# NVIDIA/DeepLearningExamples

Measured on AMD Instinct MI355X. Metric: training samples/sec, higher is better.
Workload: dtype bf16; 1 GPU; ResNet-50 v1.5 (PyTorch/Classification/ConvNets) synthetic ImageNet 224x224, label smoothing 0.1, SGD momentum 0.875 (BASELINE.json configs[1]); batch_per_gpu=256, global_batch=256, layout=NHWC, hip_graph=False, parallelism=single GPU

## Files before the change

deeplearningexamples_amd/_cabi.py:

```python
import ctypes
import os

import torch

_HERE = os.path.dirname(os.path.abspath(__file__))
LIB_PATH = os.environ.get("DLE_LIB_PATH") or os.path.join(_HERE, "lib", "libdle_mi355x.so")

F32, F16, BF16 = 0, 1, 2
ACT_NONE, ACT_RELU, ACT_GELU, ACT_RELU_BWD, ACT_ADD, ACT_GELU_BWD, ACT_TANH, ACT_TANH_BWD = 0, 1, 2, 3, 4, 5, 6, 7
ACT_ADD_MASKED, ACT_MUL, ACT_GELU_DAUX = 8, 9, 10

_DT = {torch.float32: F32, torch.float16: F16, torch.bfloat16: BF16}

c_void_p, c_int, c_i64, c_float = ctypes.c_void_p, ctypes.c_int, ctypes.c_int64, ctypes.c_float
c_u64 = ctypes.c_uint64

_SIGS = {
    "dle_last_error": (ctypes.c_char_p, []),
    "dle_abi_version": (c_int, []),
    "dle_device_check": (c_int, [c_int, ctypes.c_char_p, c_int]),
    "dle_dot_interact_out_width": (c_int, [c_int, c_int]),
    "dle_dot_interact_fwd": (c_int, [c_void_p, c_void_p, c_int, c_int, c_int, c_int, c_int, c_void_p]),
    "dle_dot_interact_bwd": (c_int, [c_void_p, c_void_p, c_void_p, c_void_p, c_int, c_int, c_int, c_int,
                                     c_int, c_void_p]),
    "dle_dot_interact_bwd_checked": (c_int, [c_void_p, c_void_p, c_void_p, c_void_p, c_int, c_int, c_int, c_int,
                                             c_int, c_void_p, c_void_p]),
    "dle_dlrm_gather_interact_try": (c_int, [c_void_p] * 6 + [c_i64, c_int, c_int, c_int, c_void_p]),
    "dle_emb_gather_fwd": (c_int, [c_void_p, c_void_p, c_void_p, c_void_p, c_void_p, c_i64, c_int, c_int,
                                   c_int, c_i64, c_void_p]),
    "dle_emb_offset_indices": (c_int, [c_void_p, c_void_p, c_void_p, c_void_p, c_i64, c_int, c_void_p]),
    "dle_emb_grad_values": (c_int, [c_void_p, c_void_p, c_void_p, c_i64, c_int, c_void_p]),
    "dle_emb_sparse_sgd": (c_int, [c_void_p, c_void_p, c_void_p, c_void_p, c_float, c_void_p, c_void_p,
                                   c_i64, c_int, c_int, c_i64, c_int, c_void_p]),
    "dle_emb_small_table_mask": (c_int, [c_void_p, c_int, c_int, c_void_p]),
    "dle_emb_sgd_dedup": (c_int, [c_void_p, c_void_p, c_void_p, c_void_p, c_void_p, c_void_p, c_void_p,
                                  c_void_p, c_float, c_void_p, c_void_p, c_i64, c_int, c_int, c_i64, c_int,
                                  c_void_p]),
    "dle_emb_sgd_dedup_ws": (c_int, [c_void_p, c_void_p, c_void_p, c_void_p, c_void_p, c_void_p, c_void_p,
                                     c_void_p, c_float, c_void_p, c_void_p, c_i64, c_int, c_int, c_i64, c_int,
                                     c_void_p, c_i64, c_void_p]),
    "dle_emb_onehot_workspace_bytes": (c_i64, [c_int, c_i64]),
    "dle_emb_sgd_workspace_bytes": (c_i64, [c_void_p, c_int, c_int, c_i64]),
    "dle_emb_onehot_try": (c_int, [c_void_p, c_void_p, c_void_p, c_void_p, c_float, c_void_p, c_void_p, c_void_p, c_void_p,
                                   c_void_p, c_int, c_i64, c_int, c_int, c_i64, c_int, c_void_p, c_i64, c_void_p]),
    "dle_emb_onehot_partials": (c_int, [c_void_p, c_void_p, c_void_p, c_void_p, c_void_p, c_void_p, c_int, c_i64, c_int, c_int,
                                        c_i64, c_int, c_void_p, c_i64, c_void_p, c_void_p]),
    "dle_emb_adam_workspace_bytes": (c_i64, [c_void_p, c_int, c_int, c_i64]),
    "dle_emb_adam_dedup_ws": (c_int, [c_void_p] * 9 + [c_float, c_void_p, c_void_p, c_void_p, c_float, c_float, c_float, c_i64,
                                      c_int, c_int, c_i64, c_int, c_void_p, c_i64, c_void_p]),
    "dle_cast_rows": (c_int, [c_void_p, c_void_p, c_i64, c_int, c_int, c_i64, c_i64, c_int, c_int, c_void_p]),
    "dle_bce_logits": (c_int, [c_void_p, c_void_p, c_void_p, c_void_p, c_void_p, c_i64, c_i64, c_int, c_void_p]),
    "dle_conv1x1_bnbwd_dgrad": (c_int, [c_void_p] * 16 + [c_i64, c_int, c_int, c_int, c_int, c_void_p]),
    "dle_conv1x1_bnbwd_groups": (c_int, [c_int]),
    "dle_conv1x1_bnbwd_dgrad_wgrad": (c_int, [c_void_p] * 15 + [c_i64, c_void_p, c_void_p, c_void_p, c_i64, c_int, c_int, c_int, c_int,
                                              c_void_p]),
    "dle_conv1x1_bnbwd_wgrad_workspace": (c_i64, [c_int, c_int]),
    "dle_gemm_expand_masked_bnred": (c_int, [c_void_p] * 10 + [c_i64, c_int, c_int, c_int, c_i64, c_i64, c_i64, c_int, c_int, c_void_p]),
    "dle_bn_bwd_finish": (c_int, [c_void_p, c_int, c_int, c_void_p, c_void_p, c_int, c_void_p]),
    "dle_gemm_colsum": (c_int, [c_void_p, c_void_p, c_void_p, c_void_p, c_void_p, c_int, c_int, c_int, c_i64, c_i64, c_i64, c_int,
                                c_int, c_int, c_void_p, c_i64, c_void_p]),
    "dle_head_bce_workspace_bytes": (c_i64, [c_i64, c_int]),
    "dle_head_bce_fwd_bwd": (c_int, [c_void_p, c_void_p, c_void_p, c_void_p, c_void_p, c_void_p, c_void_p, c_void_p, c_void_p,
                                     c_void_p, c_void_p, c_void_p, c_i64, c_i64, c_int, c_i64, c_i64, c_int, c_void_p]),
    "dle_amp_update_scale": (c_int, [c_void_p, c_void_p, c_void_p, c_void_p, c_float, c_float, c_int, c_int,
                                     c_void_p]),
    "dle_check_nonfinite": (c_int, [c_void_p, c_void_p, c_i64, c_int, c_void_p]),
    "dle_axpby_f32": (c_int, [c_void_p, c_void_p, c_void_p, c_float, c_float, c_i64, c_void_p]),
    "dle_act_bwd": (c_int, [c_void_p, c_void_p, c_void_p, c_i64, c_int, c_int, c_void_p]),
    "dle_relu_bwd": (c_int, [c_void_p, c_void_p, c_void_p, c_i64, c_int, c_i64, c_i64, c_i64, c_int, c_void_p]),
    "dle_gemm": (c_int, [c_void_p, c_void_p, c_void_p, c_void_p, c_void_p, c_void_p, c_int, c_int, c_int,
                         c_i64, c_i64, c_i64, c_int, c_int, c_int, c_int, c_int, c_int, c_int, c_float,
                         c_void_p, c_i64, c_void_p]),
    "dle_conv2d_fwd": (c_int, [c_void_p, c_void_p, c_void_p, c_void_p] + [c_int] * 12 + [c_void_p]),
    "dle_conv2d_fwd_affine": (c_int, [c_void_p] * 6 + [c_int] * 11 + [c_void_p]),
    "dle_conv3x3_affine_launch_count": (c_i64, []),
    "dle_conv2d_grouped_fwd_affine": (c_int, [c_void_p] * 5 + [c_int] * 9 + [c_void_p]),
    "dle_se_gate": (c_int, [c_void_p] * 6 + [c_int] * 5 + [c_void_p]),
    "dle_se_apply": (c_int, [c_void_p] * 4 + [c_i64, c_int, c_int, c_int, c_int, c_void_p]),
    "dle_conv2d_dgrad": (c_int, [c_void_p, c_void_p, c_void_p, c_void_p] + [c_int] * 10 + [c_void_p]),
    "dle_conv2d_wgrad": (c_int, [c_void_p, c_void_p, c_void_p] + [c_int] * 12 + [c_void_p, c_i64, c_void_p]),
    "dle_nchw_to_nhwc": (c_int, [c_void_p, c_void_p, c_i64, c_int, c_i64, c_int, c_int, c_void_p]),
    "dle_gemm_expand_add_up2": (c_int, [c_void_p, c_void_p, c_void_p, c_void_p, c_int, c_int, c_int, c_i64, c_i64, c_i64, c_i64, c_int,
                                        c_int, c_int, c_int, c_void_p]),
    "dle_conv1x1_bnload_groups": (c_int, [c_int, c_int, c_int]),
    "dle_conv1x1_bnload_fwd": (c_int, [c_void_p] * 11 + [c_i64, c_int, c_int, c_int, c_int, c_void_p]),
    "dle_bn_relu_maxpool_fwd": (c_int, [c_void_p] * 8 + [c_int, c_int, c_int, c_int, c_int, c_void_p]),
    "dle_wgrad1x1_workspace": (c_i64, []),
    "dle_wgrad1x1_mode": (c_int, [c_int]),
    "dle_wgrad1x1_workspace_for": (c_i64, [c_int, c_int, c_int]),
    "dle_gemm8_mode": (c_int, [c_int]),
    "dle_gemm8_min_items": (c_int, [c_int]),
    "dle_gemm8_launch_count": (c_i64, []),
    "dle_wgrad1x1_try": (c_int, [c_void_p, c_void_p, c_void_p, c_int, c_int, c_int, c_int, c_int, c_void_p, c_i64, c_void_p]),
    "dle_conv3x3_wgrad_workspace": (c_i64, []),
    "dle_conv3x3_wgrad_mode": (c_int, [c_int]),
    "dle_stem_conv7_groups": (c_int, [c_int, c_int]),
    "dle_stem_conv7_fwd": (c_int, [c_void_p, c_void_p, c_void_p, c_void_p, c_i64, c_int, c_int, c_int, c_int, c_void_p]),
    "dle_stem_conv7_wgrad_workspace": (c_i64, [c_int, c_int]),
    "dle_stem_conv7_wgrad": (c_int, [c_void_p, c_void_p, c_void_p, c_void_p, c_i64, c_int, c_int, c_int, c_int, c_int, c_void_p]),
    "dle_stem_pack_weight": (c_int, [c_void_p, c_void_p, c_int, c_void_p]),
    "dle_bn_workspace_bytes": (c_i64, [c_i64, c_int]),
    "dle_bn_fwd_stats": (c_int, [c_void_p, c_i64, c_int, c_float, c_float, c_void_p, c_void_p, c_void_p, c_void_p,
                                 c_void_p, c_i64, c_int, c_void_p]),
    "dle_conv2d_fwd_colstats": (c_int, [c_void_p, c_void_p, c_void_p] + [c_int] * 10 + [c_void_p, c_i64, c_void_p, c_void_p]),
    "dle_bn_stats_from_partials": (c_int, [c_void_p, c_int, c_i64, c_int, c_float, c_float, c_void_p, c_void_p, c_void_p,
                                           c_void_p, c_void_p, c_i64, c_void_p]),
    "dle_bn_fwd_apply": (c_int, [c_void_p] * 8 + [c_i64, c_int, c_int, c_int, c_void_p]),
    "dle_rccl_available": (c_int, []),
    "dle_rccl_unique_id": (c_int, [c_void_p]),
# ... 278 lines not shown
```

deeplearningexamples_amd/convnets/resnet.py:

```python
from contextlib import nullcontext as _nullcontext
from typing import List

import os

import torch
from torch import nn

from .. import _cabi as C
from .. import functional as F

LAYERS, WIDTHS, EXPANSION = [3, 4, 6, 3], [64, 128, 256, 512], 4


def _conv(cin, cout, k, stride, device):
    m = nn.Conv2d(cin, cout, kernel_size=k, stride=stride, padding=(k - 1) // 2, bias=False, device=device)
    nn.init.kaiming_normal_(m.weight, mode="fan_in", nonlinearity="relu")
    m.weight.data = m.weight.data.contiguous(memory_format=torch.channels_last)
    return m


def _bn(c, device, zero_init=False):
    m = nn.BatchNorm2d(c, device=device)
    nn.init.constant_(m.weight, 0 if zero_init else 1)
    nn.init.constant_(m.bias, 0)
    return m


class Deferred:
    __slots__ = ("unit", "t", "mean", "rstd", "residual", "y")

    def __init__(self, unit, t, mean, rstd, residual):
        self.unit, self.t, self.mean, self.rstd, self.residual, self.y = unit, t, mean, rstd, residual, None

    def residual_args(self):
        r = self.residual
        if isinstance(r, Deferred):
            return r.t, (r.mean, r.rstd, r.unit.bn.weight.data, r.unit.bn.bias.data)
        return r, None

    def _done(self, y, mask):
        u = self.unit
        u.saved = (u.saved[0], self.t, mask, self.mean, self.rstd)
        self.y = y

    def materialize(self):
        if self.y is None:
            u = self.unit
            res, res_bn = self.residual_args()
            y, mask = F.bn_fwd_apply(self.t, self.mean, self.rstd, u.bn.weight.data, u.bn.bias.data, residual=res,
                                     relu=u.relu, want_mask=True, residual_bn=res_bn)
            self._done(y, mask)
        return self.y


class ConvBN:

    def __init__(self, conv: nn.Conv2d, bn: nn.BatchNorm2d, name_conv: str, name_bn: str, relu: bool):
        self.conv, self.bn, self.name_conv, self.name_bn, self.relu = conv, bn, name_conv, name_bn, relu
        self.k = conv.kernel_size[0]
        self.stride, self.pad = conv.stride[0], conv.padding[0]
        self.cin, self.cout = conv.in_channels, conv.out_channels
        self.w16 = None
        self.gw = self.ggamma = self.gbeta = None
        self.saved = None
        self.w2 = self.gw_flat = None
        self.wgrad_stream = None
        self.fuse_bnbwd = os.environ.get("DLE_RN50_FUSE_BNBWD", "1") != "0"
        self.fuse_bnbwd_wgrad = os.environ.get("DLE_RN50_FUSE_BNBWD_WGRAD", "1") != "0"
        self.reduce_done = False
        self.keepalive = None

    def forward(self, x, residual=None, defer=False):
        t = None
        if isinstance(x, Deferred):
            d, r = x, None
            if self.k == 1 and self.stride == 1 and d.unit.relu and d.y is None:
                res, res_bn = d.residual_args()
                r = F.conv1x1_bnload_fwd(d.t, res, self.w16, d.mean, d.rstd, d.unit.bn.weight.data, d.unit.bn.bias.data,
                                         self.bn.running_mean, self.bn.running_var, eps=self.bn.eps, momentum=self.bn.momentum,
                                         res_bn=res_bn)
            if r is not None:
                t, x, bits, mean, rstd = r
                d._done(x, bits)
            else:
                x = d.materialize()
        if t is None:
            if x.shape[-1] == 4:
                t, mean, rstd = F.stem_conv_fwd_bnstats(x, self.w2, self.bn.running_mean, self.bn.running_var, eps=self.bn.eps,
                                                        momentum=self.bn.momentum)
            else:
                t, mean, rstd = F.conv2d_fwd_bnstats(x, self.w16, self.stride, self.pad, self.bn.running_mean,
                                                     self.bn.running_var, eps=self.bn.eps, momentum=self.bn.momentum)
        if defer:
            self.saved = (x, t, None, mean, rstd)
            return Deferred(self, t, mean, rstd, residual)
        if isinstance(residual, Deferred):
            d = Deferred(self, t, mean, rstd, residual)
            self.saved = (x, t, None, mean, rstd)
            return d.materialize()
        y, mask = F.bn_fwd_apply(t, mean, rstd, self.bn.weight.data, self.bn.bias.data, residual=residual,
                                 relu=self.relu, want_mask=True)
        self.saved = (x, t, mask, mean, rstd)
        return y

    def forward_eval(self, x, residual=None):
        t = F.stem_conv_fwd(x, self.w2, want_stats=False)[0] if x.shape[-1] == 4 else F.conv2d_fwd(x, self.w16, self.stride, self.pad)
        rstd = torch.rsqrt(self.bn.running_var + self.bn.eps)
        y, _ = F.bn_fwd_apply(t, self.bn.running_mean, rstd, self.bn.weight.data, self.bn.bias.data, residual=residual,
                              relu=self.relu, want_mask=False)
        return y

    def backward(self, dy, need_dx=True, dx_addend=None, dy_mask=None, compact_dx=False, bnred=None, pooled=None):
        x, t, mask, mean, rstd = self.saved
        self.saved = None
        self.saved_c = x.shape[-1]
        rmask = mask if self.relu else dy_mask
        n, h, w, c = x.shape
        reduce_done, self.reduce_done = self.reduce_done, False
        fused = None
        wgrad_done = False
        if self.fuse_bnbwd and self.k == 1 and self.stride == 1 and need_dx and dx_addend is None:
            b2 = None
            if bnred is not None and bnred.saved is not None and bnred.relu:
                b2 = (bnred.saved[1], bnred.saved[2], bnred.saved[3], bnred.saved[4], bnred.ggamma, bnred.gbeta)
            if self.fuse_bnbwd_wgrad and pooled is None and self.gw is not None:
                r = F.bn_bwd_conv1x1_dgrad_wgrad(dy, t, mean, rstd, self.bn.weight.data, self.ggamma, self.gbeta,
                                                 self.w16.view(self.cout, c), x, self.gw, relu_mask=rmask,
                                                 reduce_done=reduce_done, bnred=b2)
                if r is not None:
                    fused, wgrad_done = (None, r[0], r[1]), True
            if fused is None:
                fused = F.bn_bwd_conv1x1_dgrad(dy, t, mean, rstd, self.bn.weight.data, self.ggamma, self.gbeta,
                                               self.w16.view(self.cout, c), relu_mask=rmask, reduce_done=reduce_done, bnred=b2)
        gt = None
        if pooled is not None:
            if self.relu and not reduce_done:
                gt = F.pool_bn_bwd(pooled[0], pooled[1], t, mean, rstd, self.bn.weight.data, self.ggamma, self.gbeta, rmask)
            if gt is None:
                dy = F.maxpool_bwd(pooled[0], pooled[1], t.shape[1:3])
        if gt is not None:
            pass
        elif fused is not None:
            gt = fused[0]
            if fused[2]:
                bnred.reduce_done = True
        else:
            gt, _ = F.bn_bwd(dy, None, t, mean, rstd, self.bn.weight.data, self.ggamma, self.gbeta, relu_mask=rmask,
                             reduce_done=reduce_done)
        up2 = isinstance(dx_addend, tuple) and dx_addend[0] == "up2"
        masked = isinstance(dx_addend, tuple) and not up2
        ws = self.wgrad_stream if not wgrad_done else None
        if ws is not None:
            ws.wait_stream(torch.cuda.current_stream())
            self.keepalive.append((gt, x))
        with (torch.cuda.stream(ws) if ws is not None else _nullcontext()):
            if wgrad_done:
                pass
            elif c == 4:
                F.stem_conv_wgrad(gt, x, self.gw_flat)
            elif self.k == 1 and self.stride == 1:
                m = n * h * w
                if not F.wgrad1x1(gt.view(m, self.cout), x.view(m, c), self.gw.view(self.cout, c)):
                    F.gemm(gt.view(m, self.cout), x.view(m, c), self.cout, c, m, False, False, out=self.gw.view(self.cout, c),
                           splitk=F.pick_splitk(self.cout, c, m, target_blocks=1024))
            else:
                F.conv2d_wgrad(gt, x, (self.k, self.k), self.stride, self.pad, out=self.gw)
        dx = None
        if fused is not None:
            dx = fused[1].view(n, h, w, c)
        elif self.k == 1 and self.stride == 1:
            m = n * h * w
            g2 = gt.view(m, self.cout)
            if need_dx:
                if masked:
                    dxf = None
                    if bnred is not None and bnred.saved is not None and bnred.relu:
                        _, pt, pmask, pmean, prstd = bnred.saved
                        dxf = F.gemm_masked_add_bnred(g2, self.w16.view(self.cout, c), m, c, self.cout, dx_addend[0].view(m, c),
# ... 80 lines not shown
```

deeplearningexamples_amd/functional.py:

```python
import os

import torch

from . import _cabi as C


def dot_interact_out_width(rows, cols):
    return C.lib().dle_dot_interact_out_width(rows, cols)


def dot_interact_fwd(x, force_generic=False):
    C.require_cuda(x)
    if x.dim() != 3:
        raise ValueError("dot_interact: expected [batch, rows, cols], got %s" % (tuple(x.shape),))
    x = x.contiguous()
    b, r, c = x.shape
    out = torch.empty((b, dot_interact_out_width(r, c)), dtype=x.dtype, device=x.device)
    C.annotate(bytes=float(b) * (r * c + out.shape[1]) * x.element_size())
    C.call("dle_dot_interact_fwd", C.ptr(x), C.ptr(out), b, r, c, C.dt(x), int(force_generic), C.stream())
    return out


def dot_interact_bwd(x, upstream, force_generic=False, fuse_mlp_grad=False, grad_out=None, found_inf=None):
    C.require_cuda(x, upstream)
# ... 1041 lines not shown
        return None
    ws = _bn_ws(x.reshape(m, k))
    act_bytes = 0.125 if relu_mask is not None else 0.0
    relu_tag = "+relu" if relu_mask is not None else ""
    if not reduce_done:
        C.annotate(bytes=float(x.numel()) * (4 + act_bytes), tag="M%dxC%d%s" % (m, k, relu_tag))
        C.call("dle_bn_bwd_reduce", C.ptr(dy), None, C.ptr(relu_mask), C.ptr(x), C.ptr(mean), C.ptr(rstd), C.ptr(dgamma),
               C.ptr(dbeta), m, k, 0, C.ptr(ws), ws.numel() * 4, C.dt(x), C.stream())
    dt = None if wg else torch.empty_like(x)
    dx = torch.empty((m, n), dtype=x.dtype, device=x.device)
    t2 = bits2 = mean2 = rstd2 = part = None
    if bnred is not None and bnred[0].numel() == m * n and bnred[0].is_contiguous() and bnred[1] is not None \
            and os.environ.get("DLE_RN50_FUSE_BNRED", "1") != "0" and os.environ.get("DLE_RN50_FUSE_BNRED2", "1") != "0":
        t2, bits2, mean2, rstd2 = bnred[:4]
    groups = int(C.lib().dle_conv1x1_bnbwd_groups(m)) if wg or t2 is not None else 0
    bnred_tag = "+bnred" if t2 is not None else ""
    if wg:
        name = "dle_conv1x1_bnbwd_dgrad_wgrad"
        wg_bytes = int(C.lib().dle_conv1x1_bnbwd_wgrad_workspace(m, int(t2 is not None)))
        part_bytes = (groups * 2 * n * 4 + 15) // 16 * 16 if t2 is not None else 0
        buf = splitk_workspace(x.device, part_bytes + wg_bytes)
        part = buf[:part_bytes // 4] if t2 is not None else None
        wpart = buf[part_bytes // 4:]
        C.annotate(bytes=float(x.numel()) * (4 + act_bytes) + (dx.numel() + xin.numel()) * 2.0
                   + dx.numel() * (2.125 if t2 is not None else 0.0),
                   flops=4.0 * m * n * k, tag="bn_bwd+dgrad+wgrad %dx%dx%d%s%s" % (m, n, k, relu_tag, bnred_tag))
        args = (C.ptr(dy), C.ptr(x), C.ptr(relu_mask), C.ptr(w), C.ptr(dx), C.ptr(mean), C.ptr(rstd), C.ptr(gamma), C.ptr(dgamma),
                C.ptr(dbeta), C.ptr(t2), C.ptr(bits2), C.ptr(mean2), C.ptr(rstd2), C.ptr(part), part_bytes, C.ptr(xin), C.ptr(gw),
                C.ptr(wpart), wpart.numel() * 4, m, n, k, C.dt(x), C.stream())
    else:
        name = "dle_conv1x1_bnbwd_dgrad"
        if t2 is not None:
            part = splitk_workspace(x.device, groups * 2 * n * 4)
        C.annotate(bytes=float(x.numel()) * (6 + act_bytes) + dx.numel() * (2.0 + (2.125 if t2 is not None else 0.0)),
                   flops=2.0 * m * n * k, tag="bn_bwd+dgrad %dx%dx%d%s%s" % (m, n, k, relu_tag, bnred_tag))
        args = (C.ptr(dy), C.ptr(x), C.ptr(relu_mask), C.ptr(w), C.ptr(dt), C.ptr(dx), C.ptr(mean), C.ptr(rstd), C.ptr(gamma),
                C.ptr(dgamma), C.ptr(dbeta), C.ptr(t2), C.ptr(bits2), C.ptr(mean2), C.ptr(rstd2), C.ptr(part),
                part.numel() * 4 if part is not None else 0, m, n, k, C.dt(x), C.stream())
    rc = _timed_optional(name, getattr(C.lib(), name), args)
    if rc > 1:
        C.check(rc - 1000 if rc > 1000 else -1, name)
    if rc != 1:
        dt, _ = bn_bwd(dy, None, x, mean, rstd, gamma, dgamma, dbeta, relu_mask=relu_mask, reduce_done=True, dx_out=dt)
        gemm(dt.view(m, k), w, m, n, k, True, False, out=dx)
        if wg and not wgrad1x1(dt.view(m, k), xin.view(m, n), gw.view(k, n)):
            gemm(dt.view(m, k), xin.view(m, n), k, n, m, False, False, out=gw.view(k, n),
                 splitk=pick_splitk(k, n, m, target_blocks=1024))
        return (None if wg else dt), dx, False
    if t2 is not None:
        C.call("dle_bn_bwd_finish", C.ptr(part), groups, n, C.ptr(bnred[4]), C.ptr(bnred[5]), 0, C.stream())
    return dt, dx, t2 is not None


def bn_bwd_conv1x1_dgrad(dy, x, mean, rstd, gamma, dgamma, dbeta, w, relu_mask=None, reduce_done=False, bnred=None):
    return _bn_bwd_conv1x1(dy, x, mean, rstd, gamma, dgamma, dbeta, w, relu_mask, reduce_done, bnred)


def bn_bwd_conv1x1_dgrad_wgrad(dy, x, mean, rstd, gamma, dgamma, dbeta, w, xin, gw, relu_mask=None, reduce_done=False, bnred=None):
    out = _bn_bwd_conv1x1(dy, x, mean, rstd, gamma, dgamma, dbeta, w, relu_mask, reduce_done, bnred, xin, gw)
    return out and out[1:]


def maxpool_fwd(x, ksize=3, stride=2, pad=1):
    C.require_cuda(x)
    n, h, w, c = x.shape
    p, q = (h + 2 * pad - ksize) // stride + 1, (w + 2 * pad - ksize) // stride + 1
    y = torch.empty((n, p, q, c), dtype=x.dtype, device=x.device)
    am = torch.empty((n, p, q, c), dtype=torch.uint8, device=x.device)
    C.annotate(bytes=float(x.numel() + y.numel()) * 2 + am.numel())
    C.call("dle_maxpool_fwd", C.ptr(x), C.ptr(y), C.ptr(am), n, h, w, c, ksize, stride, pad, C.dt(x), C.stream())
    return y, am


def maxpool_bwd(dy, argmax, in_hw, ksize=3, stride=2, pad=1):
    C.require_cuda(dy, argmax)
    n, p, q, c = dy.shape
    h, w = in_hw
    dx = torch.empty((n, h, w, c), dtype=dy.dtype, device=dy.device)
    C.annotate(bytes=float(dx.numel() + dy.numel()) * 2 + argmax.numel())
    C.call("dle_maxpool_bwd", C.ptr(dy), C.ptr(argmax), C.ptr(dx), n, h, w, c, ksize, stride, pad, C.dt(dy), C.stream())
    return dx


def pool_bn_bwd(dy, argmax, x, mean, rstd, gamma, dgamma, dbeta, relu_mask):
    C.require_cuda(dy, argmax, x, mean, rstd, gamma, dgamma, dbeta, relu_mask)
    n, h, w, c = x.shape
    if relu_mask is None or dy.shape != (n, h // 2, w // 2, c) or not (dy.is_contiguous() and x.is_contiguous()) or dy.dtype != x.dtype:
        return None
    nbytes = int(C.lib().dle_pool_bn_bwd_workspace_bytes(n, h, w, c))
    if nbytes == 0:
        return None
    ws = splitk_workspace(x.device, nbytes)
    dz = torch.empty_like(x)
    C.annotate(bytes=2.0 * (dy.numel() * 3 + x.numel() * 2.125) + x.numel() * 2.0, tag="N%dx%dx%dxC%d" % (n, h, w, c))
    C.call("dle_pool_bn_bwd", C.ptr(dy), C.ptr(argmax), C.ptr(relu_mask), C.ptr(x), C.ptr(dz), C.ptr(mean), C.ptr(rstd), C.ptr(gamma),
           C.ptr(dgamma), C.ptr(dbeta), n, h, w, c, C.ptr(ws), ws.numel() * 4, C.dt(x), C.stream())
    return dz


def avgpool_fwd(x):
    C.require_cuda(x)
    n, h, w, c = x.shape
    y = torch.empty((n, c), dtype=x.dtype, device=x.device)
    C.call("dle_avgpool_fwd", C.ptr(x), C.ptr(y), n, h * w, c, C.dt(x), C.stream())
    return y


def avgpool_bwd(dy, hw):
    C.require_cuda(dy)
    n, c = dy.shape
    h, w = hw
# ... 624 lines not shown
```

include/dle_mi355x.h:

```cpp
#ifndef DLE_MI355X_H
#define DLE_MI355X_H
#include <stdint.h>

#ifdef __cplusplus
extern "C" {
#endif

typedef struct ihipStream_t* hipStream_t;

enum { DLE_F32 = 0, DLE_F16 = 1, DLE_BF16 = 2 };
enum { DLE_ACT_NONE = 0, DLE_ACT_RELU = 1, DLE_ACT_GELU = 2, DLE_ACT_RELU_BWD = 3, DLE_ACT_ADD = 4,
       DLE_ACT_GELU_BWD = 5, DLE_ACT_TANH = 6, DLE_ACT_TANH_BWD = 7,
       DLE_ACT_ADD_MASKED = 8,
       DLE_ACT_MUL = 9,
       DLE_ACT_GELU_DAUX = 10   };

const char* dle_last_error(void);
int dle_abi_version(void);
int dle_device_check(int device, char* arch_name, int arch_name_len);

int dle_dot_interact_out_width(int rows, int cols);
int dle_dot_interact_fwd(const void* x, void* out, int batch, int rows, int cols, int dtype,
                         int force_generic, hipStream_t stream);
int dle_dot_interact_bwd(const void* x, const void* upstream, void* grad, void* mlp_grad,
// ... 137 lines not shown
                         int clear_found_inf, hipStream_t stream);
int dle_check_nonfinite(const void* x, float* found_inf, int64_t n, int dtype, hipStream_t stream);
int dle_axpby_f32(const float* x, const float* y, float* out, float a, float b, int64_t n, hipStream_t stream);
int dle_act_bwd(const void* g, const void* src, void* out, int64_t n, int act, int dtype, hipStream_t stream);
int dle_relu_bwd(const void* g, const void* y, void* out, int64_t rows, int cols, int64_t ld_g, int64_t ld_y,
                 int64_t ld_out, int dtype, hipStream_t stream);

int dle_nchw_to_nhwc(const float* x, void* y, int64_t N, int C, int64_t HW, int C_padded, int out_dtype,
                     hipStream_t stream);
int64_t dle_bn_workspace_bytes(int64_t M, int C);
int dle_bn_fwd_stats(const void* x, int64_t M, int C, float eps, float momentum, float* mean, float* rstd,
                     float* running_mean, float* running_var, void* workspace, int64_t workspace_bytes,
                     int dtype, hipStream_t stream);
int dle_conv2d_fwd_colstats(const void* x, const void* w, void* y, int N, int H, int W, int C, int Ko, int R, int S,
                            int stride, int pad, int dtype, float* col_partial, int64_t col_partial_bytes,
                            int* groups, hipStream_t stream);
int dle_bn_stats_from_partials(const float* partial, int groups, int64_t M, int C, float eps, float momentum,
                               float* mean, float* rstd, float* running_mean, float* running_var, void* workspace,
                               int64_t workspace_bytes, hipStream_t stream);
int dle_bn_fwd_apply(const void* x, const void* residual, void* y, void* relu_mask, const float* mean,
                     const float* rstd, const float* gamma, const float* beta, int64_t M, int C, int relu,
                     int dtype, hipStream_t stream);
int dle_bn_fwd_apply2(const void* x, const void* xr, void* y, void* relu_mask, const float* mean, const float* rstd,
                      const float* gamma, const float* beta, const float* mean_r, const float* rstd_r, const float* gamma_r,
                      const float* beta_r, int64_t M, int C, int dtype, hipStream_t stream);
int dle_bn_bwd_reduce(const void* dy, const void* y, const void* relu_mask, const void* x, const float* mean,
                      const float* rstd, float* dgamma, float* dbeta, int64_t M, int C, int accumulate,
                      void* workspace, int64_t workspace_bytes, int dtype, hipStream_t stream);
int dle_bn_bwd_reduce2(const void* dy, const void* relu_mask, const void* x1, const float* mean1, const float* rstd1, float* dgamma1,
                       float* dbeta1, const void* x2, const float* mean2, const float* rstd2, float* dgamma2, float* dbeta2,
                       int64_t M, int C, void* workspace, int64_t workspace_bytes, int dtype, hipStream_t stream);
int dle_bn_bwd_apply(const void* dy, const void* y, const void* relu_mask, const void* x, void* dx, void* g_out,
                     const float* mean, const float* rstd, const float* gamma, const float* dgamma,
                     const float* dbeta, int64_t M, int C, int dtype, hipStream_t stream);
int dle_conv1x1_bnload_groups(int M, int N, int K);
int dle_conv1x1_bnload_fwd(const void* t, const void* res, const void* w, void* out, void* y, void* bits, const float* mean,
                           const float* rstd, const float* gamma, const float* beta, float* stats, int64_t stats_bytes, int M,
                           int N, int K, int dtype, hipStream_t stream);
int dle_conv1x1_bnload_fwd2(const void* t, const void* res, const void* w, void* out, void* y, void* bits, const float* mean,
                            const float* rstd, const float* gamma, const float* beta, const float* mean_r, const float* rstd_r,
                            const float* gamma_r, const float* beta_r, float* stats, int64_t stats_bytes, int M, int N, int K,
                            int dtype, hipStream_t stream);
int dle_conv1x1_bnbwd_dgrad(const void* dy, const void* t, const void* relu_mask, const void* w, void* dt, void* dx,
                            const float* mean, const float* rstd, const float* gamma, const float* dgamma, const float* dbeta,
                            const void* t2, const void* bits2, const float* mean2, const float* rstd2, float* partial,
                            int64_t partial_bytes, int M, int N, int K, int dtype, hipStream_t stream);
int dle_conv1x1_bnbwd_groups(int M);
int dle_conv1x1_bnbwd_dgrad_wgrad(const void* dy, const void* t, const void* relu_mask, const void* w, void* dx,
                                  const float* mean, const float* rstd, const float* gamma, const float* dgamma,
                                  const float* dbeta, const void* t2, const void* bits2, const float* mean2, const float* rstd2,
                                  float* partial, int64_t partial_bytes, const void* x, float* gw, void* workspace,
                                  int64_t workspace_bytes, int M, int N, int K, int dtype, hipStream_t stream);
int64_t dle_conv1x1_bnbwd_wgrad_workspace(int M, int bnred);
int dle_gemm_expand_masked_bnred(const void* A, const void* B, void* C, const void* src, const void* bits, const void* t2,
                                 const void* bits2, const float* mean2, const float* rstd2, float* partial, int64_t partial_bytes,
                                 int M, int N, int K, int64_t lda, int64_t ldb, int64_t ldc, int b_kc, int dtype, hipStream_t stream);
int dle_bn_bwd_finish(const float* partial, int groups, int C, float* dgamma, float* dbeta, int accumulate, hipStream_t stream);
int dle_stem_conv7_groups(int N, int H);
int dle_stem_conv7_fwd(const void* x4, const void* w2, void* y, float* stats, int64_t stats_bytes, int N, int H, int W,
                       int dtype, hipStream_t stream);
int64_t dle_stem_conv7_wgrad_workspace(int N, int H);
int dle_stem_conv7_wgrad(const void* dy, const void* x4, float* dw, void* workspace, int64_t workspace_bytes, int N, int H,
                         int W, int dtype, int accumulate, hipStream_t stream);
int dle_stem_pack_weight(const float* w_krsc, void* out, int dtype, hipStream_t stream);
int dle_maxpool_fwd(const void* x, void* y, void* argmax, int N, int H, int W, int C, int ksize, int stride,
                    int pad, int dtype, hipStream_t stream);
int dle_bn_relu_maxpool_fwd(const void* x, void* y, void* argmax, void* relu_mask, const float* mean, const float* rstd,
                            const float* gamma, const float* beta, int N, int H, int W, int C, int dtype, hipStream_t stream);
int dle_maxpool_bwd(const void* dy, const void* argmax, void* dx, int N, int H, int W, int C, int ksize,
                    int stride, int pad, int dtype, hipStream_t stream);
int64_t dle_pool_bn_bwd_workspace_bytes(int N, int H, int W, int C);
int dle_pool_bn_bwd(const void* dy, const void* argmax, const void* relu_mask, const void* x, void* dz, const float* mean,
                    const float* rstd, const float* gamma, float* dgamma, float* dbeta, int N, int H, int W, int C, void* workspace,
                    int64_t workspace_bytes, int dtype, hipStream_t stream);
int dle_avgpool_fwd(const void* x, void* y, int64_t N, int HW, int C, int dtype, hipStream_t stream);
int dle_avgpool_bwd(const void* dy, void* dx, int64_t N, int HW, int C, int dtype, hipStream_t stream);
int dle_gemm_expand_add_up2(const void* A, const void* B, void* C, const void* compact, int M, int N, int K, int64_t lda,
                            int64_t ldb, int64_t ldc, int64_t ld_compact, int b_kc, int H, int W, int dtype, hipStream_t stream);
int dle_upsample_zero(const void* x, void* y, int64_t N, int P, int Q, int H, int W, int C, int stride, int dtype,
                      hipStream_t stream);
int dle_softmax_xent(const float* logits, const int64_t* target, float* loss_out, void* dlogits,
                     const float* grad_scale_dev, int* scratch, int64_t rows, int classes, int64_t ld,
                     int64_t ld_out, float smoothing, int64_t ignore_index, int dlogits_dtype,
                     hipStream_t stream);

int dle_layernorm_fwd(const void* x, const void* residual, void* z_out, void* y, const float* gamma,
                      const float* beta, float* mean, float* rstd, int64_t rows, int H, float eps, int dtype,
                      hipStream_t stream);
int64_t dle_layernorm_workspace_bytes(int H);
int dle_layernorm_bwd(const void* dy, const void* z, const float* mean, const float* rstd, const float* gamma,
                      void* dz, float* dgamma, float* dbeta, int64_t rows, int H, int accumulate, void* workspace,
                      int64_t workspace_bytes, int dtype, hipStream_t stream);
int dle_embed_sum(const float* word, const float* pos, const float* type, const int64_t* ids,
                  const int64_t* token_type, void* z, int64_t tokens, int S, int H, int dtype, hipStream_t stream);
int dle_embed_sum_packed(const float* word, const float* pos, const float* type, const int64_t* ids,
                         const int64_t* token_type, const int32_t* position_ids, void* z, int64_t tokens, int H, int dtype,
                         hipStream_t stream);
int dle_embed_scatter_add(const void* dz, const int64_t* ids, float* grad_word, int64_t tokens, int H, int dtype,
                          hipStream_t stream);
int dle_rows_select_sum(const void* x, const int64_t* sel, float* out, int64_t rows, int H, int K, int accumulate,
                        void* workspace, int64_t workspace_bytes, int dtype, hipStream_t stream);
int dle_rows_gather(const void* src, const int64_t* idx, void* dst, int64_t n, int H, int dtype, hipStream_t stream);
int dle_rows_scatter(const void* src, const int64_t* idx, void* dst, int64_t n, int H, int accumulate, int dtype,
                     hipStream_t stream);
int dle_softmax_fwd(void* scores, const float* mask_add, int64_t rows, int L, int rows_per_batch, float scale,
                    int dtype, hipStream_t stream);
// ... 185 lines not shown
```

Baseline: 13360 samples/s.

## Add fused BN-backward dgrad+wgrad kernel for 512x128 1x1 convs

Adds a dedicated HIP kernel that fuses the BN backward elementwise step with both the data-gradient and weight-gradient GEMMs for 1x1 convs of shape K=512, N=128. It uses LDS transpose reads, DMA into LDS and MFMA, and writes per-block weight-gradient partials that are then folded. It is meant to avoid materialising the BN-backward output and extra passes over activations. By default the S2 env flag is off, so this shape now bypasses the existing fused wgrad path and uses the separate path instead.

```diff
diff --git a/deeplearningexamples_amd/_cabi.py b/deeplearningexamples_amd/_cabi.py
--- a/deeplearningexamples_amd/_cabi.py
+++ b/deeplearningexamples_amd/_cabi.py
@@ -55,6 +55,9 @@
     "dle_conv1x1_bnbwd_dgrad_wgrad": (c_int, [c_void_p] * 15 + [c_i64, c_void_p, c_void_p, c_void_p, c_i64, c_int, c_int, c_int, c_int,
                                               c_void_p]),
     "dle_conv1x1_bnbwd_wgrad_workspace": (c_i64, [c_int, c_int]),
+    "dle_conv1x1_bnbwd_wg512": (c_int, [c_void_p] * 13 + [c_i64, c_int, c_int, c_int, c_int, c_void_p]),
+    "dle_conv1x1_bnbwd_wg512_groups": (c_int, [c_int]),
+    "dle_conv1x1_bnbwd_wg512_workspace": (c_i64, [c_int]),
     "dle_gemm_expand_masked_bnred": (c_int, [c_void_p] * 10 + [c_i64, c_int, c_int, c_int, c_i64, c_i64, c_i64, c_int, c_int, c_void_p]),
     "dle_bn_bwd_finish": (c_int, [c_void_p, c_int, c_int, c_void_p, c_void_p, c_int, c_void_p]),
     "dle_gemm_colsum": (c_int, [c_void_p, c_void_p, c_void_p, c_void_p, c_void_p, c_int, c_int, c_int, c_i64, c_i64, c_i64, c_int,
diff --git a/deeplearningexamples_amd/convnets/resnet.py b/deeplearningexamples_amd/convnets/resnet.py
--- a/deeplearningexamples_amd/convnets/resnet.py
+++ b/deeplearningexamples_amd/convnets/resnet.py
@@ -67,6 +67,7 @@
         self.wgrad_stream = None
         self.fuse_bnbwd = os.environ.get("DLE_RN50_FUSE_BNBWD", "1") != "0"
         self.fuse_bnbwd_wgrad = os.environ.get("DLE_RN50_FUSE_BNBWD_WGRAD", "1") != "0"
+        self.fuse_bnbwd_wgrad_s2 = os.environ.get("DLE_RN50_FUSE_BNBWD_WGRAD_S2", "0") != "0"
         self.reduce_done = False
         self.keepalive = None
 
@@ -123,7 +124,8 @@
             b2 = None
             if bnred is not None and bnred.saved is not None and bnred.relu:
                 b2 = (bnred.saved[1], bnred.saved[2], bnred.saved[3], bnred.saved[4], bnred.ggamma, bnred.gbeta)
-            if self.fuse_bnbwd_wgrad and pooled is None and self.gw is not None:
+            wg_on = self.fuse_bnbwd_wgrad and ((self.cout, c) != (512, 128) or self.fuse_bnbwd_wgrad_s2)
+            if wg_on and pooled is None and self.gw is not None:
                 r = F.bn_bwd_conv1x1_dgrad_wgrad(dy, t, mean, rstd, self.bn.weight.data, self.ggamma, self.gbeta,
                                                  self.w16.view(self.cout, c), x, self.gw, relu_mask=rmask,
                                                  reduce_done=reduce_done, bnred=b2)
diff --git a/deeplearningexamples_amd/csrc/conv_bnbwd_wg512.hip b/deeplearningexamples_amd/csrc/conv_bnbwd_wg512.hip
--- /dev/null
+++ b/deeplearningexamples_amd/csrc/conv_bnbwd_wg512.hip
@@ -0,0 +1,277 @@
+#include "gemm_tiles.h"
+
+struct Wg5Args {
+  const unsigned short* DY;
+  const unsigned short* T;
+  const unsigned char* bits;
+  const unsigned short* W;
+  const unsigned short* X;
+  unsigned short* DX;
+  float* ws;
+  const float* mean; const float* rstd; const float* gamma; const float* dgamma; const float* dbeta;
+  float inv_m;
+  int M, ntiles;
+};
+
+#define G5_K 512
+#define G5_N 128
+#define G5_TG 32
+#define G5_LG (G5_K * 2)
+#define G5_LX (G5_N * 2)
+#define G5_DT_OFF 0
+#define G5_X_OFF (G5_TG * G5_LG)
+#define G5_XBYTES (G5_TG * G5_LX)
+#define G5_W_OFF (G5_X_OFF + 2 * G5_XBYTES)
+#define G5_WROWS 128
+#define G5_WBYTES (G5_WROWS * G5_LX)
+#define G5_CF_OFF (G5_W_OFF + 2 * G5_WBYTES)
+#define G5_LDS_BYTES (G5_CF_OFF + 5 * G5_K * 4)
+#define G5_MAX_GROUPS 256
+
+template <int OFF>
+__device__ __forceinline__ short4_t g5_tr(unsigned addr) {
+  short4_t v;
+  asm volatile("ds_read_b64_tr_b16 %0, %1 offset:%2" : "=v"(v) : "v"(addr), "n"(OFF) : "memory");
+  return v;
+}
+
+__device__ __forceinline__ int g5_swz(int r) { return ((r & 3) << 2) | ((r >> 2) & 3); }
+__device__ __forceinline__ int g5_xswz(int r) { return r & 3; }
+
+__device__ __forceinline__ void g5_dma16_soff(int4v_t rs, unsigned short* lds_wave_base, unsigned voff, int soff) {
+  const int m0v = __builtin_amdgcn_readfirstlane((int)(unsigned)(__UINTPTR_TYPE__)(lds_void*)lds_wave_base);
+  const int so = __builtin_amdgcn_readfirstlane(soff);
+  asm volatile("s_mov_b32 m0, %0\n\ts_nop 0\n\tbuffer_load_dwordx4 %1, %2, %3 offen lds" :: "s"(m0v), "v"(voff), "s"(rs), "s"(so) : "memory");
+}
+
+template <int DT, bool MASK>
+__global__ __launch_bounds__(512) void conv_bnbwd_wg512_kernel(Wg5Args p) {
+  constexpr int K = G5_K, LG = G5_LG, LX = G5_LX;
+  extern __shared__ __attribute__((aligned(16))) unsigned char smem_raw[];
+  const int tid = threadIdx.x, lane = tid & 63, wave = tid >> 6;
+  const int wave_u = __builtin_amdgcn_readfirstlane(wave);
+  float* cf = (float*)(smem_raw + G5_CF_OFF);
+  for (int c = tid; c < K; c += 512) {
+    const float rs = p.rstd[c];
+    cf[c] = p.gamma[c] * rs;
+    cf[K + c] = p.mean[c];
+    cf[2 * K + c] = rs;
+    cf[3 * K + c] = p.dbeta[c] * p.inv_m;
+    cf[4 * K + c] = p.dgamma[c] * p.inv_m;
+  }
+  const int4v_t rx = rsrc_words(p.X), rw = rsrc_words(p.W);
+
+  const int dma_r = lane >> 4, dma_cb = (lane & 15) * 16;
+  const unsigned dma_lane = (unsigned)(dma_r * LX + (((dma_cb >> 6) ^ g5_xswz(dma_r)) << 6) + (dma_cb & 63));
+  auto issue_x = [&](int t, int buf) __attribute__((always_inline)) {
+    const long long m = (long long)t * G5_TG + wave_u * 4 + dma_r;
+    dma16_raw(rx, (unsigned short*)(smem_raw + G5_X_OFF + buf * G5_XBYTES + wave_u * 1024),
+              m < p.M ? (unsigned)((m - dma_r) * LX) + dma_lane : OOB_OFF);
+  };
+  auto issue_w = [&](int chunk, int slot) __attribute__((always_inline)) {
+#pragma unroll
+    for (int k = 0; k < 4; ++k) {
+      const int pc = wave_u + 8 * k;
+      g5_dma16_soff(rw, (unsigned short*)(smem_raw + G5_W_OFF + slot * G5_WBYTES + pc * 1024), dma_lane,
+                    (chunk * G5_WROWS + pc * 4) * LX);
+    }
+  };
+
+  ushort8_t gq[4], tq[4];
+  unsigned mq[4];
+  auto load_rows = [&](int t) __attribute__((always_inline)) {
+#pragma unroll
+    for (int i = 0; i < 4; ++i) {
+      const long long m = (long long)t * G5_TG + wave + 8 * i;
+      const unsigned mr = (unsigned)(m < p.M ? m : p.M - 1);
+      const unsigned o = mr * (unsigned)LG + (unsigned)lane * 16u;
+      gq[i] = *(const ushort8_t*)((const unsigned char*)p.DY + o);
+      tq[i] = *(const ushort8_t*)((const unsigned char*)p.T + o);
+      mq[i] = MASK ? (unsigned)p.bits[mr * (unsigned)(K / 8) + (unsigned)lane] : 0xffu;
+    }
+  };
+
+  float16_t acc[2][4];
+#pragma unroll
+  for (int i = 0; i < 2; ++i)
+#pragma unroll
+    for (int j = 0; j < 4; ++j)
+#pragma unroll
+      for (int r = 0; r < 16; ++r) acc[i][j][r] = 0.f;
+
+  const unsigned lds0 = (unsigned)(unsigned long)(__attribute__((address_space(3))) unsigned char*)smem_raw;
+  const int tg = lane >> 4, ti = lane & 15;
+  const int r0 = (tg >> 1) * 8 + (ti >> 2);
+  const int chanb = ((tg & 1) * 16 + (ti & 3) * 4) * 2;
+  const int c16 = wave * 8 + (chanb >> 4);
+  const unsigned alo_ = (unsigned)(r0 * LG + ((c16 ^ g5_swz(r0)) << 4) + (chanb & 15));
+  const unsigned ahi_ = (unsigned)((r0 + 4) * LG + ((c16 ^ g5_swz(r0 + 4)) << 4) + (chanb & 15));
+  const unsigned boff_ = (unsigned)(r0 * LX + (g5_xswz(r0) << 6) + chanb);
+  const unsigned woff_ = lds0 + G5_W_OFF + (unsigned)(r0 * LX + (((wave & 3) ^ g5_xswz(r0)) << 6) + chanb);
+  const int fr = lane & 31, fh = lane >> 5;
+  const unsigned doff_ = (unsigned)(fr * LG + ((fh ^ g5_swz(fr)) << 4));
+
+  int t = blockIdx.x, it = 0;
+  load_rows(t);
+  issue_x(t, 0);
+  issue_w(0, 0);
+  __syncthreads();
+  for (; t < p.ntiles; t += gridDim.x, ++it) {
+    const int xb = it & 1;
+    unsigned alo = alo_, ahi = ahi_, boff = boff_, woff = woff_, doff = doff_;
+    asm volatile("" : "+v"(alo), "+v"(ahi), "+v"(boff), "+v"(woff), "+v"(doff));
+    const int tn = t + (int)gridDim.x;
+    __builtin_amdgcn_s_waitcnt(0x0F70);
+    lds_barrier();
+#pragma unroll
+    for (int h = 0; h < 2; ++h) {
+      float ka[4], kmu[4], krs[4], kb[4], kgm[4];
+      const int c0 = lane * 8 + 4 * h;
+#pragma unroll
+      for (int k = 0; k < 4; ++k) {
+        ka[k] = cf[c0 + k]; kmu[k] = cf[K + c0 + k]; krs[k] = cf[2 * K + c0 + k];
+        kb[k] = cf[3 * K + c0 + k]; kgm[k] = cf[4 * K + c0 + k];
+      }
+#pragma unroll
+      for (int i = 0; i < 4; ++i) {
+        float gf[8], xf[8], of[8];
+        unpack8<DT>(gq[i], gf);
+        unpack8<DT>(tq[i], xf);
+        const unsigned bits = mq[i] >> (4 * h);
+#pragma unroll
+        for (int k = 0; k < 4; ++k) {
+          float g = gf[4 * h + k];
+          if (MASK) { if (!((bits >> k) & 1u)) g = 0.f; }
+          const float xh = (xf[4 * h + k] - kmu[k]) * krs[k];
+          of[k] = ka[k] * (g - kb[k] - xh * kgm[k]);
+          of[4 + k] = 0.f;
+        }
+        const uint4_t o = __builtin_bit_cast(uint4_t, pack8<DT>(of));
+        const int r = wave + 8 * i;
+        const bool live = (long long)t * G5_TG + r < p.M;
+        *(uint2_t*)(smem_raw + G5_DT_OFF + r * LG + ((lane ^ g5_swz(r)) << 4) + 8 * h) = live ? (uint2_t){o[0], o[1]} : (uint2_t){0u, 0u};
+      }
+    }
+    if (tn < p.ntiles) {
+      load_rows(tn);
+      issue_x(tn, xb ^ 1);
+    }
+    lds_barrier();
+    {
+      const unsigned xo = lds0 + G5_X_OFF + (unsigned)(xb * G5_XBYTES);
+      static_for<0, G5_TG / 16>([&](auto KS) __attribute__((always_inline)) {
+        constexpr int ks = decltype(KS)::value;
+        TrPair fa[2], fb[4];
+#pragma unroll
+        for (int i = 0; i < 2; ++i) { fa[i].lo = g5_tr<ks * 16 * LG>(lds0 + G5_DT_OFF + (alo ^ (unsigned)(i << 6))); fa[i].hi = g5_tr<ks * 16 * LG>(lds0 + G5_DT_OFF + (ahi ^ (unsigned)(i << 6))); }
+#pragma unroll
+        for (int j = 0; j < 4; ++j) { const unsigned a = xo + (boff ^ (unsigned)(j << 6)); fb[j].lo = g5_tr<ks * 16 * LX>(a); fb[j].hi = g5_tr<ks * 16 * LX + 4 * LX>(a); }
+        frag_wait<true>();
+#pragma unroll
+        for (int i = 0; i < 2; ++i) {
+          const ushort8_t va = frag_value(fa[i]);
+#pragma unroll
+          for (int j = 0; j < 4; ++j) acc[i][j] = Mfma32x16<DT>::run(va, frag_value(fb[j]), acc[i][j]);
+        }
+      });
+    }
+    float16_t dacc;
+#pragma unroll
+    for (int r = 0; r < 16; ++r) dacc[r] = 0.f;
+    static_for<0, 4>([&](auto CH) __attribute__((always_inline)) {
+      constexpr int ch = decltype(CH)::value, slot = ch & 1;
+      if constexpr (ch > 0) {
+        __builtin_amdgcn_s_waitcnt(0x0F70);
+        lds_barrier();
+      }
+      issue_w((ch + 1) & 3, slot ^ 1);
+      if (wave_u < 4) {
+        static_for<0, 8>([&](auto KS) __attribute__((always_inline)) {
+          constexpr int ks = decltype(KS)::value;
+          TrPair fw;
+          fw.lo = g5_tr<slot * G5_WBYTES + ks * 16 * LX>(woff);
+          fw.hi = g5_tr<slot * G5_WBYTES + ks * 16 * LX + 4 * LX>(woff);
+          const ushort8_t fd = *(const ushort8_t*)(smem_raw + G5_DT_OFF + ch * 256 + (doff ^ (unsigned)(ks << 5)));
+          frag_wait<true>();
+          dacc = Mfma32x16<DT>::run(frag_value(fw), fd, dacc);
+        });
+      }
+    });
+    unsigned char* stg = smem_raw + G5_X_OFF + xb * G5_XBYTES;
+    if (wave_u < 4) {
+      float v[16];
+#pragma unroll
+      for (int r = 0; r < 16; ++r) v[r] = dacc[r];
+      const ushort8_t o0 = pack8<DT>(v), o1 = pack8<DT>(v + 8);
+      const uint4_t u0 = __builtin_bit_cast(uint4_t, o0), u1 = __builtin_bit_cast(uint4_t, o1);
+#pragma unroll
+      for (int q = 0; q < 4; ++q) {
+        const int nb = (32 * wave + 8 * q + 4 * fh) * 2;
+        const uint2_t w2 = q == 0 ? (uint2_t){u0[0], u0[1]} : q == 1 ? (uint2_t){u0[2], u0[3]}
+                         : q == 2 ? (uint2_t){u1[0], u1[1]} : (uint2_t){u1[2], u1[3]};
+        *(uint2_t*)(stg + fr * LX + (((nb >> 4) ^ (fr & 15)) << 4) + (nb & 15)) = w2;
+      }
+    }
+    lds_barrier();
+    {
+      const int row = tid >> 4, cc = tid & 15;
+      const uint4_t ov = *(const uint4_t*)(stg + row * LX + ((cc ^ (row & 15)) << 4));
+      const long long m = (long long)t * G5_TG + row;
+      if (m < p.M) *(uint4_t*)(p.DX + m * G5_N + cc * 8) = ov;
+    }
+  }
+  __builtin_amdgcn_s_waitcnt(0x0F70);
+  float* out = p.ws + (long long)blockIdx.x * (G5_K * G5_N);
+#pragma unroll
+  for (int i = 0; i < 2; ++i)
+#pragma unroll
+    for (int j = 0; j < 4; ++j) {
+      const int c = j * 32 + (lane & 31);
+#pragma unroll
+      for (int r = 0; r < 16; ++r) {
+        const int ko = (wave * 2 + i) * 32 + 8 * (r >> 2) + 4 * (lane >> 5) + (r & 3);
+        out[ko * G5_N + c] = acc[i][j][r];
+      }
+    }
+}
+
+extern "C" int dle_conv1x1_bnbwd_wg512_groups(int M) {
+  if (M <= 0) return 0;
+  const int ntiles = (M + G5_TG - 1) / G5_TG;
+  return ntiles < G5_MAX_GROUPS ? ntiles : G5_MAX_GROUPS;
+}
+
+extern "C" int64_t dle_conv1x1_bnbwd_wg512_workspace(int M) {
+  return (int64_t)dle_conv1x1_bnbwd_wg512_groups(M) * G5_K * G5_N * 4;
+}
+
+extern "C" int dle_conv1x1_bnbwd_wg512(const void* dy, const void* t, const void* relu_mask, const void* w, void* dx,
+                                       const float* mean, const float* rstd, const float* gamma, const float* dgamma,
+                                       const float* dbeta, const void* x, float* gw, void* workspace, int64_t workspace_bytes,
+                                       int M, int N, int K, int dtype, hipStream_t stream) {
+  if (dtype != DLE_F16 && dtype != DLE_BF16) return 0;
+  if (K != G5_K || N != G5_N || M < 8192 || (long long)M * G5_LG >= 0xFFFFFFE0LL) return 0;
+  if (!dy || !t || !w || !dx || !mean || !rstd || !gamma || !dgamma || !dbeta || !x || !gw || !workspace) return 0;
+  if (((((uintptr_t)dy) | ((uintptr_t)t) | ((uintptr_t)w) | ((uintptr_t)dx) | ((uintptr_t)relu_mask) | ((uintptr_t)x) |
+        ((uintptr_t)gw) | ((uintptr_t)workspace)) & 15) != 0)
+    return 0;
+  if (workspace_bytes < dle_conv1x1_bnbwd_wg512_workspace(M)) return 0;
+  static const int on = dle_env_int("DLE_CONV_BNBWD", 1);
+  if (!on) return 0;
+  Wg5Args p;
+  p.DY = (const unsigned short*)dy; p.T = (const unsigned short*)t; p.bits = (const unsigned char*)relu_mask;
+  p.W = (const unsigned short*)w; p.X = (const unsigned short*)x; p.DX = (unsigned short*)dx; p.ws = (float*)workspace;
+  p.mean = mean; p.rstd = rstd; p.gamma = gamma; p.dgamma = dgamma; p.dbeta = dbeta; p.inv_m = 1.0f / (float)M;
+  p.M = M; p.ntiles = (M + G5_TG - 1) / G5_TG;
+  const int groups = dle_conv1x1_bnbwd_wg512_groups(M);
+  const dim3 grid((unsigned)groups), block(512);
+#define G5_GO(DT) do { if (relu_mask) DLE_LAUNCH_LDS((conv_bnbwd_wg512_kernel<DT, true>), grid, block, G5_LDS_BYTES, stream, p); \
+                       else DLE_LAUNCH_LDS((conv_bnbwd_wg512_kernel<DT, false>), grid, block, G5_LDS_BYTES, stream, p); } while (0)
+  if (dtype == DLE_F16) G5_GO(DLE_F16); else G5_GO(DLE_BF16);
+#undef G5_GO
+  hipError_t e = hipGetLastError();
+  if (e != hipSuccess) { dle_set_error("conv1x1_bnbwd_wg512 launch failed: %s", hipGetErrorString(e)); return (int)e + 1000; }
+  e = wgrad1x1_fold((const float*)workspace, gw, (long long)G5_K * G5_N / 4, groups, 0, stream);
+  if (e != hipSuccess) { dle_set_error("conv1x1_bnbwd_wg512 fold launch failed: %s", hipGetErrorString(e)); return (int)e + 1000; }
+  return 1;
+}
diff --git a/deeplearningexamples_amd/functional.py b/deeplearningexamples_amd/functional.py
--- a/deeplearningexamples_amd/functional.py
+++ b/deeplearningexamples_amd/functional.py
@@ -1117,11 +1117,51 @@
     return dt, dx, t2 is not None
 
 
+def _bn_bwd_conv1x1_wg512(dy, x, mean, rstd, gamma, dgamma, dbeta, w, relu_mask, reduce_done, xin, gw):
+    C.require_cuda(dy, x, mean, rstd, gamma, dgamma, dbeta, w, relu_mask, xin, gw)
+    k = x.shape[-1]
+    m = x.numel() // k
+    n = w.shape[-1]
+    if (k != 512 or n != 128 or m < 4096 or w.numel() != k * n or not all(t.is_contiguous() for t in (dy, x, w, xin, gw))
+            or x.dtype not in (torch.float16, torch.bfloat16) or dy.dtype != x.dtype or w.dtype != x.dtype or xin.dtype != x.dtype
+            or dy.numel() != m * k or xin.numel() != m * n or gw.numel() != k * n or gw.dtype != torch.float32
+            or os.environ.get("DLE_CONV_BNBWD", "1") == "0"
+            or any(t is not None and t.data_ptr() % 16 for t in (dy, x, w, relu_mask, xin, gw))):
+        return None
+    ws = _bn_ws(x.reshape(m, k))
+    act_bytes = 0.125 if relu_mask is not None else 0.0
+    relu_tag = "+relu" if relu_mask is not None else ""
+    if not reduce_done:
+        C.annotate(bytes=float(x.numel()) * (4 + act_bytes), tag="M%dxC%d%s" % (m, k, relu_tag))
+        C.call("dle_bn_bwd_reduce", C.ptr(dy), None, C.ptr(relu_mask), C.ptr(x), C.ptr(mean), C.ptr(rstd), C.ptr(dgamma),
+               C.ptr(dbeta), m, k, 0, C.ptr(ws), ws.numel() * 4, C.dt(x), C.stream())
+    dx = torch.empty((m, n), dtype=x.dtype, device=x.device)
+    wpart = splitk_workspace(x.device, max(int(C.lib().dle_conv1x1_bnbwd_wg512_workspace(m)), 16))
+    C.annotate(bytes=float(x.numel()) * (4 + act_bytes) + (dx.numel() + xin.numel()) * 2.0, flops=4.0 * m * n * k,
+               tag="bn_bwd+dgrad+wgrad %dx%dx%d%s" % (m, n, k, relu_tag))
+    name = "dle_conv1x1_bnbwd_wg512"
+    rc = _timed_optional(name, C.lib().dle_conv1x1_bnbwd_wg512,
+                         (C.ptr(dy), C.ptr(x), C.ptr(relu_mask), C.ptr(w), C.ptr(dx), C.ptr(mean), C.ptr(rstd), C.ptr(gamma),
+                          C.ptr(dgamma), C.ptr(dbeta), C.ptr(xin), C.ptr(gw), C.ptr(wpart), wpart.numel() * 4, m, n, k, C.dt(x),
+                          C.stream()))
+    if rc > 1:
+        C.check(rc - 1000 if rc > 1000 else -1, name)
+    if rc != 1:
+        dt, _ = bn_bwd(dy, None, x, mean, rstd, gamma, dgamma, dbeta, relu_mask=relu_mask, reduce_done=True)
+        gemm(dt.view(m, k), w, m, n, k, True, False, out=dx)
+        if not wgrad1x1(dt.view(m, k), xin.view(m, n), gw.view(k, n)):
+            gemm(dt.view(m, k), xin.view(m, n), k, n, m, False, False, out=gw.view(k, n),
+                 splitk=pick_splitk(k, n, m, target_blocks=1024))
+    return dx, False
+
+
 def bn_bwd_conv1x1_dgrad(dy, x, mean, rstd, gamma, dgamma, dbeta, w, relu_mask=None, reduce_done=False, bnred=None):
     return _bn_bwd_conv1x1(dy, x, mean, rstd, gamma, dgamma, dbeta, w, relu_mask, reduce_done, bnred)
 
 
 def bn_bwd_conv1x1_dgrad_wgrad(dy, x, mean, rstd, gamma, dgamma, dbeta, w, xin, gw, relu_mask=None, reduce_done=False, bnred=None):
+    if x.shape[-1] == 512 and w.shape[-1] == 128:
+        return _bn_bwd_conv1x1_wg512(dy, x, mean, rstd, gamma, dgamma, dbeta, w, relu_mask, reduce_done, xin, gw)
     out = _bn_bwd_conv1x1(dy, x, mean, rstd, gamma, dgamma, dbeta, w, relu_mask, reduce_done, bnred, xin, gw)
     return out and out[1:]
 
diff --git a/include/dle_mi355x.h b/include/dle_mi355x.h
--- a/include/dle_mi355x.h
+++ b/include/dle_mi355x.h
@@ -213,6 +213,12 @@
                                   float* partial, int64_t partial_bytes, const void* x, float* gw, void* workspace,
                                   int64_t workspace_bytes, int M, int N, int K, int dtype, hipStream_t stream);
 int64_t dle_conv1x1_bnbwd_wgrad_workspace(int M, int bnred);
+int dle_conv1x1_bnbwd_wg512(const void* dy, const void* t, const void* relu_mask, const void* w, void* dx, const float* mean,
+                            const float* rstd, const float* gamma, const float* dgamma, const float* dbeta, const void* x,
+                            float* gw, void* workspace, int64_t workspace_bytes, int M, int N, int K, int dtype,
+                            hipStream_t stream);
+int dle_conv1x1_bnbwd_wg512_groups(int M);
+int64_t dle_conv1x1_bnbwd_wg512_workspace(int M);
 int dle_gemm_expand_masked_bnred(const void* A, const void* B, void* C, const void* src, const void* bits, const void* t2,
                                  const void* bits2, const float* mean2, const float* rstd2, float* partial, int64_t partial_bytes,
                                  int M, int N, int K, int64_t lda, int64_t ldb, int64_t ldc, int b_kc, int dtype, hipStream_t stream);
```

Measured after the change: 13300 samples/s. About the same (-0.4%).
